# Kiripiro/leaffliction

Hardware: AMD Instinct MI355X
Metric: 224x224 images/sec train (higher is better)
Workload: dtype f32; 1 GPU; leaf_cnn base train step (configs[1]: img 224, batch 256/GPU, fp32, 8 classes, AdamW+clipnorm+EMA, in-model augmentation); per_gpu_batch=256, global_batch=256, img_size=224, parallelism=dp1

## Files before the change

leaffliction_amd/csrc/lf_conv.hip:

```cpp
#include <type_traits>

#include "lf_common.h"

namespace {

typedef float f32x16 __attribute__((ext_vector_type(16)));
typedef float f32x4 __attribute__((ext_vector_type(4)));

constexpr int kThreads = 256;

__device__ __forceinline__ float pro_apply(float v, float sc, float sh, int relu) {
    v = fmaf(v, sc, sh);
    return relu ? fmaxf(v, 0.f) : v;
}

typedef float lf_f4 __attribute__((ext_vector_type(4)));
constexpr unsigned kBufOob = 0xffffffffu;
__device__ __forceinline__ __amdgpu_buffer_rsrc_t buf_rsrc(const float* base, unsigned bytes) {
    return __builtin_amdgcn_make_buffer_rsrc(const_cast<float*>(base), 0, bytes, 0x00020000);
}
__device__ __forceinline__ float4 buf_load4(__amdgpu_buffer_rsrc_t r, unsigned off) {
    const lf_f4 v = __builtin_bit_cast(lf_f4, __builtin_amdgcn_raw_buffer_load_b128(r, off, 0, 0));
    return make_float4(v.x, v.y, v.z, v.w);
}
__device__ __forceinline__ float buf_load1(__amdgpu_buffer_rsrc_t r, unsigned off) {
    return __builtin_bit_cast(float, __builtin_amdgcn_raw_buffer_load_b32(r, off, 0, 0));
}

struct ConvArgs {
    const float* x;
    const float* w;
    const float* wino_u;
    float* y;
    const float* in_scale;
    const float* in_shift;
    int n, cin, cout, h, wd;
    int tiles_x, tiles_y;
    int in_relu;
    int accumulate;
    int vec_ok;
    int stack;
    float* stat_part;
    const float* stat_pivot;
    long long stat_tiles;
    const float* stat_mask_y;
    const float* mask_scale;
    const float* mask_shift;
    int mask_relu;
};

using lf::half_sum32;
using lf::row_sum16;

__device__ __forceinline__ void wino_filter(const float (&g)[9], float (&u)[16]) {
    float t[4][3];
#pragma unroll
    for (int c = 0; c < 3; ++c) {
        const float s = g[c] + g[6 + c];
        t[0][c] = g[c];
        t[1][c] = (s + g[3 + c]) * 0.5f;
        t[2][c] = (s - g[3 + c]) * 0.5f;
        t[3][c] = g[6 + c];
    }
#pragma unroll
    for (int r = 0; r < 4; ++r) {
        const float s = t[r][0] + t[r][2];
        u[r * 4 + 0] = t[r][0];
        u[r * 4 + 1] = (s + t[r][1]) * 0.5f;
        u[r * 4 + 2] = (s - t[r][1]) * 0.5f;
        u[r * 4 + 3] = t[r][2];
    }
}
__device__ __forceinline__ void wino_input(const float (&d)[16], float (&v)[16]) {
    float t[16];
#pragma unroll
    for (int c = 0; c < 4; ++c) {
        t[0 + c] = d[0 + c] - d[8 + c];
        t[4 + c] = d[4 + c] + d[8 + c];
        t[8 + c] = d[8 + c] - d[4 + c];
        t[12 + c] = d[4 + c] - d[12 + c];
    }
#pragma unroll
    for (int r = 0; r < 4; ++r) {
        v[r * 4 + 0] = t[r * 4 + 0] - t[r * 4 + 2];
        v[r * 4 + 1] = t[r * 4 + 1] + t[r * 4 + 2];
        v[r * 4 + 2] = t[r * 4 + 2] - t[r * 4 + 1];
        v[r * 4 + 3] = t[r * 4 + 1] - t[r * 4 + 3];
    }
}
__device__ __forceinline__ void wino_output(const float (&m)[16], float (&y)[4]) {
    float b[2][4];
#pragma unroll
    for (int c = 0; c < 4; ++c) {
        b[0][c] = m[0 + c] + m[4 + c] + m[8 + c];
        b[1][c] = m[4 + c] - m[8 + c] - m[12 + c];
    }
#pragma unroll
    for (int r = 0; r < 2; ++r) {
        y[r * 2 + 0] = b[r][0] + b[r][1] + b[r][2];
        y[r * 2 + 1] = b[r][1] - b[r][2] - b[r][3];
    }
}

constexpr int kMaxProC = 512;

template <int TW, int TH, int HALO, bool STK>
struct ConvTile {
    int bz, by, tile;
    int tx0, ty0, n;
    int imgA, gyA0, ra;
    bool imgA_ok, imgB_ok;

    __device__ __forceinline__ explicit ConvTile(const ConvArgs& p) {
        const unsigned gxy = gridDim.x * gridDim.y, gtotal = gxy * gridDim.z;
        const unsigned bflat = blockIdx.x + gridDim.x * (blockIdx.y + gridDim.y * blockIdx.z);
        const unsigned xk = bflat & 7u, xfloor = gtotal >> 3, xrem = gtotal & 7u;
        const unsigned wid_flat = xk * xfloor + (xk < xrem ? xk : xrem) + (bflat >> 3);
        bz = (int)(wid_flat / gxy);
        by = (int)((wid_flat - (unsigned)bz * gxy) / gridDim.x);
        tile = (int)(wid_flat - (unsigned)bz * gxy - (unsigned)by * gridDim.x);
        tx0 = (tile % p.tiles_x) * TW;
        ty0 = (tile / p.tiles_x) * TH;
        n = bz * p.stack;
        imgA = ty0 / p.h;
        gyA0 = ty0 - imgA * p.h;
        ra = min(TH, p.h - gyA0);
        imgA_ok = imgA < p.stack && n + imgA < p.n;
        imgB_ok = STK && imgA + 1 < p.stack && n + imgA + 1 < p.n;
    }

    __device__ __forceinline__ bool patch_row(int py, int h, int& img, int& gy) const {
        if (py < ra + 2 * HALO) {
            img = imgA;
            gy = gyA0 - HALO + py;
            return imgA_ok && gy >= 0 && gy < h;
        }
        img = imgA + 1;
        gy = py - (ra + 2 * HALO) - HALO;
        return imgB_ok && ra < TH && gy >= 0 && gy < h && gy < TH - ra + HALO;
    }
};

template <int TW, int TH, int HALO, bool STK, int kKC>
struct PatchStage {
    static constexpr int PW = TW + 2 * HALO, PH = TH + 2 * HALO + (STK ? 2 * HALO : 0), PP = PW * PH;
    static constexpr int TW4 = TW / 4;
    static constexpr int NVI = kKC * PH * TW4, IPT = (NVI + kThreads - 1) / kThreads;
    static constexpr int NHI = kKC * PH * 2 * HALO, HPT = (NHI + kThreads - 1) / kThreads;
    static_assert(TW % 4 == 0, "float4 patch rows");

    size_t hw;
    float4 pv[IPT];
    float ph[HPT > 0 ? HPT : 1];
    unsigned pg[IPT], pl[IPT];
    unsigned hg[HPT > 0 ? HPT : 1], hl[HPT > 0 ? HPT : 1];
    unsigned okmask = 0;

    __device__ __forceinline__ PatchStage(const ConvArgs& p, const ConvTile<TW, TH, HALO, STK>& t, float* lsc, int tid) {
        if (p.in_scale != nullptr) {
            for (int c = tid; c < p.cin && c < kMaxProC; c += kThreads) {
                lsc[c] = p.in_scale[c];
                lsc[kMaxProC + c] = p.in_shift[c];
            }
        }
        hw = (size_t)p.h * p.wd;
        const unsigned uhw = (unsigned)hw;
#pragma unroll
        for (int i = 0; i < IPT; ++i) {
            const int e = tid + i * kThreads;
            const int kc = e / (PH * TW4), rem = e - kc * (PH * TW4);
            const int py = rem / TW4, slot = rem - py * TW4;
            int img, gy;
            const bool ok = t.patch_row(py, p.h, img, gy) && e < NVI;
            pg[i] = ok ? 4u * ((unsigned)(img * p.cin + kc) * uhw + (unsigned)gy * (unsigned)p.wd + (unsigned)(t.tx0 + 4 * slot)) : kBufOob;
            pl[i] = (unsigned)(kc * PP + py * PW + HALO + 4 * slot) | ((unsigned)kc << 16);
            okmask |= (ok ? 1u : 0u) << i;
        }
#pragma unroll
        for (int i = 0; i < HPT; ++i) {
            const int e = tid + i * kThreads;
            const int kc = e / (PH * 2), rem = e - kc * (PH * 2);
            const int py = rem >> 1, side = rem & 1;
            const int gx = side ? t.tx0 + TW : t.tx0 - 1;
            int img, gy;
            const bool ok = t.patch_row(py, p.h, img, gy) && e < NHI && gx >= 0 && gx < p.wd;
            hg[i] = ok ? 4u * ((unsigned)(img * p.cin + kc) * uhw + (unsigned)gy * (unsigned)p.wd + (unsigned)gx) : kBufOob;
            hl[i] = (unsigned)(kc * PP + py * PW + (side ? PW - 1 : 0)) | ((unsigned)kc << 16);
            okmask |= (ok ? 1u : 0u) << (16 + i);
        }
    }

    __device__ __forceinline__ void load(const ConvArgs& p, const float* xin, int c0) {
        const __amdgpu_buffer_rsrc_t rx = buf_rsrc(
            xin + (size_t)c0 * hw,
            4u * (unsigned)((STK ? (p.stack - 1) * p.cin : 0) + min(kKC, p.cin - c0)) * (unsigned)hw);
#pragma unroll
        for (int i = 0; i < IPT; ++i) pv[i] = buf_load4(rx, pg[i]);
#pragma unroll
        for (int i = 0; i < HPT; ++i) ph[i] = buf_load1(rx, hg[i]);
    }

    __device__ __forceinline__ void store(const ConvArgs& p, float* lp, const float* lsc, int c0, int tid) const {
        const bool pro = p.in_scale != nullptr;
        auto pro_sc = [&](int c) { return c < kMaxProC ? lsc[c] : p.in_scale[c]; };
        auto pro_sh = [&](int c) { return c < kMaxProC ? lsc[kMaxProC + c] : p.in_shift[c]; };
#pragma unroll
        for (int i = 0; i < IPT; ++i) {
            if (tid + i * kThreads < NVI) {
                const int kc = (int)(pl[i] >> 16);
                float4 v = pv[i];
                if (pro && (okmask >> i & 1u)) {
                    const float sc = pro_sc(c0 + kc), sh = pro_sh(c0 + kc);
                    v.x = pro_apply(v.x, sc, sh, p.in_relu);
                    v.y = pro_apply(v.y, sc, sh, p.in_relu);
                    v.z = pro_apply(v.z, sc, sh, p.in_relu);
                    v.w = pro_apply(v.w, sc, sh, p.in_relu);
                }
                float* dst = lp + (pl[i] & 0xffffu);
                dst[0] = v.x;
                dst[1] = v.y;
                dst[2] = v.z;
                dst[3] = v.w;
            }
        }
#pragma unroll
        for (int i = 0; i < HPT; ++i) {
            if (tid + i * kThreads < NHI) {
                const int kc = (int)(hl[i] >> 16);
                float v = ph[i];
                if (pro && (okmask >> (16 + i) & 1u))
                    v = pro_apply(v, pro_sc(c0 + kc), pro_sh(c0 + kc), p.in_relu);
                lp[hl[i] & 0xffffu] = v;
            }
        }
    }

    static __device__ __forceinline__ void stage_scalar(const ConvArgs& p, float* lp, const float* xin,
                                                        int tx0, int ty0, int c0, int tid) {
        constexpr int SLOTS = PP <= 64 ? 64 : (PP <= 128 ? 128 : 256);
        constexpr int G = kThreads / SLOTS;
        constexpr int ROUNDS = (PP + SLOTS - 1) / SLOTS;
        const int slot = tid % SLOTS, grp = tid / SLOTS;
        const size_t hw = (size_t)p.h * p.wd;
        const unsigned uhw = (unsigned)hw;
        const bool pro = p.in_scale != nullptr;
#pragma unroll
        for (int r = 0; r < ROUNDS; ++r) {
            const int pos = slot + r * SLOTS;
            if (pos < PP) {
                const int py = pos / PW, px = pos - py * PW;
                const int gy = ty0 + py - HALO, gx = tx0 + px - HALO;
                const bool inb = gy >= 0 && gy < p.h && gx >= 0 && gx < p.wd;
                const unsigned goff = inb ? (unsigned)gy * (unsigned)p.wd + (unsigned)gx : 0u;
#pragma unroll 4
                for (int kc = grp; kc < kKC; kc += G) {
                    const int c = c0 + kc;
                    float v = 0.f;
                    if (inb && c < p.cin) {
                        v = xin[(unsigned)c * uhw + goff];
                        if (pro) v = pro_apply(v, p.in_scale[c], p.in_shift[c], p.in_relu);
                    }
                    lp[kc * PP + pos] = v;
                }
            }
        }
    }
};

template <int WPX, int CT>
__device__ __forceinline__ void write_stat_part(const ConvArgs& p, const float* red, int bz, int tile, int co0,
                                                int tid) {
    __syncthreads();
    const long long tg = (long long)bz * (p.tiles_x * p.tiles_y) + tile;
    for (int c = tid; c < CT; c += kThreads) {
        if (co0 + c >= p.cout) continue;
        float a = 0.f, b = 0.f;
#pragma unroll
        for (int wp = 0; wp < WPX; ++wp) {
            a += red[(wp * CT + c) * 2];
            b += red[(wp * CT + c) * 2 + 1];
        }
        float* dst = p.stat_part + ((size_t)(co0 + c) * (size_t)p.stat_tiles + (size_t)tg) * 2;
        dst[0] = a;
        dst[1] = b;
    }
}

template <int TAPS, int TW, int TH, int WCO, int MB, int WPX, int NB, int kKC, bool STK = false>
__global__ __launch_bounds__(kThreads, (MB * NB * 16 <= 32 ? 3 : 2))
void conv_mfma_kernel(ConvArgs p) {
    constexpr int NPB = TW * TH / 32;
    static_assert(TW * TH % 32 == 0, "tile must be whole 32-pixel blocks");
    static_assert(WCO * WPX == 4 && WPX * NB == NPB, "wave decomposition");
    constexpr int CT = 32 * WCO * MB;
    constexpr int HALO = TAPS == 9 ? 1 : 0;
    using Patch = PatchStage<TW, TH, HALO, STK, kKC>;
    constexpr int PW = Patch::PW, PP = Patch::PP;
    constexpr int PATCH = kKC * PP;
    constexpr int WSZ = kKC * TAPS * CT;
    static_assert(PATCH % 4 == 0, "16-byte aligned weight region");
    constexpr int CT4 = CT / 4, NWI = kKC * TAPS * CT4, WPT = (NWI + kThreads - 1) / kThreads;

    __shared__ __attribute__((aligned(16))) float lds[PATCH + WSZ];
    __shared__ float lsc[2 * kMaxProC];
    float* lp = lds;
    float* lw = lds + PATCH;

    const int tid = threadIdx.x, lane = tid & 63, wid = tid >> 6;
    const int wave_co = wid % WCO, wave_px = wid / WCO;
    const ConvTile<TW, TH, HALO, STK> t(p);
    const int co0 = t.by * CT;
    const size_t hw = (size_t)p.h * p.wd;
    const unsigned uhw = (unsigned)hw;
    const float* xin = p.x + (size_t)t.n * p.cin * hw;

    const int khalf = lane >> 5, j = lane & 31;
    int bbase[NB];
#pragma unroll
    for (int nb = 0; nb < NB; ++nb) {
        const int f = (wave_px * NB + nb) * 32 + j;
        const int r = f / TW, prow = (STK && r >= t.ra) ? r + 2 * HALO : r;
        bbase[nb] = khalf * PP + prow * PW + (f % TW);
    }
    const int abase = khalf * TAPS * CT + wave_co * MB * 32 + j;

    f32x16 acc[MB][NB];
#pragma unroll
    for (int m = 0; m < MB; ++m)
#pragma unroll
        for (int nb = 0; nb < NB; ++nb)
#pragma unroll
            for (int r = 0; r < 16; ++r) acc[m][nb][r] = 0.f;

    auto compute_chunk = [&]() {
#pragma unroll 2
        for (int cp = 0; cp < kKC / 2; ++cp) {
            const float* lwc = lw + abase + 2 * cp * TAPS * CT;
            const float* lpc = lp + 2 * cp * PP;
#pragma unroll
            for (int tap = 0; tap < TAPS; ++tap) {
                const int dy = TAPS == 9 ? tap / 3 : 0, dx = TAPS == 9 ? tap % 3 : 0;
                float a[MB], b[NB];
#pragma unroll
                for (int m = 0; m < MB; ++m) a[m] = lwc[tap * CT + m * 32];
#pragma unroll
                for (int nb = 0; nb < NB; ++nb) b[nb] = lpc[bbase[nb] + dy * PW + dx];
#pragma unroll
                for (int m = 0; m < MB; ++m)
#pragma unroll
                    for (int nb = 0; nb < NB; ++nb)
                        acc[m][nb] = __builtin_amdgcn_mfma_f32_32x32x2f32(a[m], b[nb], acc[m][nb], 0, 0, 0);
            }
        }
    };

    const int nchunks = (p.cin + kKC - 1) / kKC;
    const bool vec = p.vec_ok && (t.tx0 + TW <= p.wd);

    if (vec) {
        float4 wv[WPT];
        constexpr bool kPrefetchW = MB * NB * 16 <= 64;
        Patch patch(p, t, lsc, tid);
        unsigned wg[WPT];
#pragma unroll
        for (int i = 0; i < WPT; ++i) {
            const int e = tid + i * kThreads;
            const int row = e / CT4, col = (e - row * CT4) * 4;
            wg[i] = (e < NWI && co0 + col < p.cout) ? 4u * ((unsigned)row * (unsigned)p.cout + (unsigned)(co0 + col)) : kBufOob;
        }
        auto load_weights = [&](int c0) {
            const __amdgpu_buffer_rsrc_t rw =
                buf_rsrc(p.w + (size_t)c0 * TAPS * p.cout,
                         4u * (unsigned)(min(kKC, p.cin - c0) * TAPS) * (unsigned)p.cout);
#pragma unroll
            for (int i = 0; i < WPT; ++i) wv[i] = buf_load4(rw, wg[i]);
        };
        auto store_chunk = [&](int c0) {
            if (!kPrefetchW) load_weights(c0);
            patch.store(p, lp, lsc, c0, tid);
#pragma unroll
            for (int i = 0; i < WPT; ++i) {
                const int e = tid + i * kThreads;
                if (e < NWI) reinterpret_cast<float4*>(lw)[e] = wv[i];
            }
        };
        patch.load(p, xin, 0);
        if (kPrefetchW) load_weights(0);
        for (int ch = 0; ch < nchunks; ++ch) {
            __syncthreads();
            store_chunk(ch * kKC);
            __syncthreads();
            if (ch + 1 < nchunks) {
                patch.load(p, xin, (ch + 1) * kKC);
                if (kPrefetchW) load_weights((ch + 1) * kKC);
            }
            compute_chunk();
        }
    } else {
        constexpr int WROWS = kKC * TAPS, RPP = kThreads / CT;
        const int wcol = tid % CT, wrow0 = tid / CT;
        const bool wcol_ok = co0 + wcol < p.cout;
        for (int ch = 0; ch < nchunks; ++ch) {
            const int c0 = ch * kKC;
            __syncthreads();
            Patch::stage_scalar(p, lp, xin, t.tx0, t.ty0, c0, tid);
            const int wvalid = (p.cin - c0) * TAPS;
#pragma unroll 4
            for (int row = wrow0; row < WROWS; row += RPP) {
                float v = 0.f;
                if (wcol_ok && row < wvalid)
                    v = p.w[((unsigned)c0 * TAPS + row) * (unsigned)p.cout + (unsigned)(co0 + wcol)];
                lw[row * CT + wcol] = v;
            }
            __syncthreads();
            compute_chunk();
        }
    }

    float* yout = p.y + (size_t)t.n * p.cout * hw;
    const bool stats = p.stat_part != nullptr, masked = p.stat_mask_y != nullptr;
    float* red = lds;
    static_assert(WPX * CT * 2 <= PATCH + WSZ, "stat scratch must fit the staging LDS");
    if (stats) __syncthreads();
    const float* my = masked ? p.stat_mask_y + (size_t)t.n * p.cout * hw : nullptr;
    constexpr int RG = TAPS == 1 ? (NB <= 2 ? 4 : 1) : (NB <= 2 ? 16 : 4);
    bool pix_ok[NB];
    unsigned pixc[NB];
#pragma unroll
    for (int nb = 0; nb < NB; ++nb) {
        const int f = (wave_px * NB + nb) * 32 + j;
        const int r = f / TW, ox = t.tx0 + f % TW;
        const bool in_a = r < t.ra;
        const int oy = in_a ? t.gyA0 + r : r - t.ra;
        pix_ok[nb] = (in_a ? t.imgA_ok : t.imgB_ok) && oy < p.h && ox < p.wd;
        pixc[nb] = pix_ok[nb] ? (unsigned)((in_a ? t.imgA : t.imgA + 1) * p.cout) * uhw +
                                    (unsigned)oy * (unsigned)p.wd + (unsigned)ox
                              : 0u;
    }
#pragma unroll
    for (int m = 0; m < MB; ++m) {
#pragma unroll
        for (int rg = 0; rg < 16; rg += RG) {
            float oldv[RG][NB], yv[RG][NB];
            if (p.accumulate) {
#pragma unroll
                for (int rr = 0; rr < RG; ++rr) {
                    const int r = rg + rr;
                    const int co = co0 + (wave_co * MB + m) * 32 + 4 * khalf + (r & 3) + 8 * (r >> 2);
                    const float* src = yout + (size_t)min(co, p.cout - 1) * hw;
#pragma unroll
                    for (int nb = 0; nb < NB; ++nb) oldv[rr][nb] = src[pixc[nb]];
                }
            }
            if (masked) {
#pragma unroll
                for (int rr = 0; rr < RG; ++rr) {
                    const int r = rg + rr;
                    const int co = co0 + (wave_co * MB + m) * 32 + 4 * khalf + (r & 3) + 8 * (r >> 2);
                    const float* src = my + (size_t)min(co, p.cout - 1) * hw;
#pragma unroll
                    for (int nb = 0; nb < NB; ++nb) yv[rr][nb] = src[pixc[nb]];
                }
            }
#pragma unroll
            for (int rr = 0; rr < RG; ++rr) {
                const int r = rg + rr;
                const int cl = (wave_co * MB + m) * 32 + 4 * khalf + (r & 3) + 8 * (r >> 2);
                const int co = co0 + cl;
                const bool co_ok = co < p.cout;
                float* dst = yout + (size_t)co * hw;
#pragma unroll
                for (int nb = 0; nb < NB; ++nb) {
                    if (p.accumulate) acc[m][nb][r] += oldv[rr][nb];
                    if (co_ok && pix_ok[nb])
                        dst[pixc[nb]] = acc[m][nb][r];
                }
                if (!stats) continue;
                float s1 = 0.f, s2 = 0.f;
                if (!masked) {
                    const float pv = (p.stat_pivot != nullptr && co_ok) ? p.stat_pivot[co] : 0.f;
#pragma unroll
                    for (int nb = 0; nb < NB; ++nb)
                        lf::stat_accumulate(acc[m][nb][r], pix_ok[nb], false, pv, 0.f, 0.f, 0.f, 0, s1, s2);
                } else {
                    const float msc = p.mask_scale[min(co, p.cout - 1)], msh = p.mask_shift[min(co, p.cout - 1)];
#pragma unroll
                    for (int nb = 0; nb < NB; ++nb)
                        lf::stat_accumulate(acc[m][nb][r], co_ok && pix_ok[nb], true, 0.f, yv[rr][nb], msc, msh,
                                            p.mask_relu, s1, s2);
                }
                s1 = half_sum32(s1);
                s2 = half_sum32(s2);
                if (j == 31) {
                    red[(wave_px * CT + cl) * 2] = s1;
                    red[(wave_px * CT + cl) * 2 + 1] = s2;
                }
            }
        }
    }
    if (stats) write_stat_part<WPX, CT>(p, red, t.bz, t.tile, co0, tid);
}

template <int TW, int TH, int MB, int NB, bool STK>
__global__ __launch_bounds__(kThreads, 2)
void conv_wino_kernel(ConvArgs p) {
    constexpr int kKC = 8, WPX = 4;
    constexpr int TXN = TW / 2, NT = TXN * (TH / 2);
    static_assert(TH % 2 == 0, "F(2x2,3x3): even tile");
    static_assert(WPX * NB * 16 >= NT, "wave decomposition");
    constexpr int CT = 16 * MB;
    constexpr int kUP = 20;
    using Patch = PatchStage<TW, TH, 1, STK, kKC>;
    constexpr int PW = Patch::PW, PP = Patch::PP;
    constexpr int PATCH = kKC * PP;
    constexpr int WSZ = kKC * CT * kUP;
    static_assert(PATCH % 4 == 0, "16-byte aligned U region");

    __shared__ __attribute__((aligned(16))) float lds[PATCH + WSZ];
    __shared__ float lsc[2 * kMaxProC];
    float* lp = lds;
    float* lw = lds + PATCH;

    const int tid = threadIdx.x, lane = tid & 63, wave_px = tid >> 6;
    const ConvTile<TW, TH, 1, STK> t(p);
    const int co0 = t.by * CT;
    const size_t hw = (size_t)p.h * p.wd;
    const unsigned uhw = (unsigned)hw;
    const float* xin = p.x + (size_t)t.n * p.cin * hw;

    const int wq = lane >> 4, wl = lane & 15;
    int vbase[NB];
    const int ubase = (wq * CT + wl) * kUP;
    f32x4 wacc[MB][NB][16];
#pragma unroll
    for (int nb = 0; nb < NB; ++nb) {
        const int tt = min((wave_px * NB + nb) * 16 + wl, NT - 1);
        const int r0 = 2 * (tt / TXN), prow = (STK && r0 >= t.ra) ? r0 + 2 : r0;
        vbase[nb] = wq * PP + prow * PW + 2 * (tt % TXN);
    }
#pragma unroll
    for (int m = 0; m < MB; ++m)
#pragma unroll
        for (int nb = 0; nb < NB; ++nb)
#pragma unroll
            for (int q = 0; q < 16; ++q) wacc[m][nb][q] = f32x4{0.f, 0.f, 0.f, 0.f};

    auto compute_chunk = [&]() {
#pragma unroll
        for (int s = 0; s < kKC / 4; ++s) {
            float u[MB][16];
#pragma unroll
            for (int m = 0; m < MB; ++m) {
                const float4* us = reinterpret_cast<const float4*>(lw + ubase + (4 * s * CT + m * 16) * kUP);
#pragma unroll
                for (int q4 = 0; q4 < 4; ++q4) {
                    const float4 v4 = us[q4];
                    u[m][4 * q4 + 0] = v4.x;
                    u[m][4 * q4 + 1] = v4.y;
                    u[m][4 * q4 + 2] = v4.z;
                    u[m][4 * q4 + 3] = v4.w;
                }
            }
#pragma unroll
            for (int nb = 0; nb < NB; ++nb) {
                const float* src = lp + vbase[nb] + 4 * s * PP;
                float d[16], v[16];
#pragma unroll
                for (int r = 0; r < 4; ++r) {
                    const float2 lo = *reinterpret_cast<const float2*>(src + r * PW);
                    const float2 hi = *reinterpret_cast<const float2*>(src + r * PW + 2);
                    d[r * 4 + 0] = lo.x;
                    d[r * 4 + 1] = lo.y;
                    d[r * 4 + 2] = hi.x;
                    d[r * 4 + 3] = hi.y;
                }
                wino_input(d, v);
#pragma unroll
                for (int m = 0; m < MB; ++m)
#pragma unroll
                    for (int q = 0; q < 16; ++q)
                        wacc[m][nb][q] = __builtin_amdgcn_mfma_f32_16x16x4f32(u[m][q], v[q], wacc[m][nb][q], 0, 0, 0);
            }
        }
    };

    constexpr int KSTEP = kThreads / (4 * CT), UPT = kKC / KSTEP;
    static_assert(kThreads % (4 * CT) == 0 && kKC % KSTEP == 0, "whole channels per pass");
    const int ukc = tid / (4 * CT), uco = (tid >> 2) % CT, uq4 = tid & 3;
    const unsigned ustep = 64u * KSTEP * (unsigned)p.cout;
    const unsigned ugo = co0 + uco < p.cout ? 4u * (((unsigned)ukc * (unsigned)p.cout + (unsigned)(co0 + uco)) * 16u + 4u * (unsigned)uq4) : 0x80000000u;
    float* const ulds = lw + (ukc * CT + uco) * kUP + 4 * uq4;
    float4 uv[UPT];
    auto load_u = [&](int c0) {
        const __amdgpu_buffer_rsrc_t ru =
            buf_rsrc(p.wino_u + (size_t)c0 * p.cout * 16, 64u * (unsigned)min(kKC, p.cin - c0) * (unsigned)p.cout);
#pragma unroll
        for (int i = 0; i < UPT; ++i) uv[i] = buf_load4(ru, ugo + (unsigned)i * ustep);
    };
    auto store_u = [&]() {
#pragma unroll
        for (int i = 0; i < UPT; ++i) *reinterpret_cast<float4*>(ulds + i * KSTEP * CT * kUP) = uv[i];
    };

    const int nchunks = (p.cin + kKC - 1) / kKC;
    const bool vec = p.vec_ok && (t.tx0 + TW <= p.wd);

    if (vec) {
        Patch patch(p, t, lsc, tid);
        patch.load(p, xin, 0);
        for (int ch = 0; ch < nchunks; ++ch) {
            __syncthreads();
            load_u(ch * kKC);
            patch.store(p, lp, lsc, ch * kKC, tid);
            store_u();
            __syncthreads();
            if (ch + 1 < nchunks) patch.load(p, xin, (ch + 1) * kKC);
            compute_chunk();
        }
    } else {
        for (int ch = 0; ch < nchunks; ++ch) {
            const int c0 = ch * kKC;
            __syncthreads();
            Patch::stage_scalar(p, lp, xin, t.tx0, t.ty0, c0, tid);
            load_u(c0);
            store_u();
            __syncthreads();
            compute_chunk();
        }
    }

    float* yout = p.y + (size_t)t.n * p.cout * hw;
    const bool stats = p.stat_part != nullptr, masked = p.stat_mask_y != nullptr;
    float* red = lds;
    static_assert(WPX * CT * 2 <= PATCH + WSZ, "stat scratch must fit the staging LDS");
    if (stats) __syncthreads();
    const float* my = masked ? p.stat_mask_y + (size_t)t.n * p.cout * hw : nullptr;
    const bool y2 = (p.wd & 1) == 0 && (reinterpret_cast<size_t>(p.y) & 7) == 0;
    bool pok[NB][4];
    unsigned pofs[NB][4];
#pragma unroll
    for (int nb = 0; nb < NB; ++nb) {
        const int tt = (wave_px * NB + nb) * 16 + wl;
        const int r0 = 2 * (tt / TXN), ox = t.tx0 + 2 * (tt % TXN);
        const bool in_a = r0 < t.ra;
        const int oy = in_a ? t.gyA0 + r0 : r0 - t.ra;
        const bool img_ok = tt < NT && (in_a ? t.imgA_ok : t.imgB_ok);
        const unsigned base = (unsigned)((in_a ? t.imgA : t.imgA + 1) * p.cout) * uhw;
#pragma unroll
        for (int q = 0; q < 4; ++q) {
            const int py = oy + (q >> 1), px = ox + (q & 1);
            pok[nb][q] = img_ok && py < p.h && px < p.wd;
            pofs[nb][q] = pok[nb][q] ? base + (unsigned)py * (unsigned)p.wd + (unsigned)px : 0u;
        }
    }
#pragma unroll
    for (int m = 0; m < MB; ++m) {
#pragma unroll
        for (int i = 0; i < 4; ++i) {
            const int cl = m * 16 + 4 * wq + i;
            const int co = co0 + cl;
            const bool co_ok = co < p.cout;
            const size_t cofs = (size_t)min(co, p.cout - 1) * hw;
            float out[NB][4], oldv[NB][4], yv[NB][4];
#pragma unroll
            for (int nb = 0; nb < NB; ++nb) {
                float mm[16];
#pragma unroll
                for (int q = 0; q < 16; ++q) mm[q] = wacc[m][nb][q][i];
                wino_output(mm, out[nb]);
                if (p.accumulate) {
#pragma unroll
                    for (int q = 0; q < 4; ++q) oldv[nb][q] = yout[cofs + pofs[nb][q]];
                }
                if (masked) {
#pragma unroll
                    for (int q = 0; q < 4; ++q) yv[nb][q] = my[cofs + pofs[nb][q]];
                }
            }
#pragma unroll
            for (int nb = 0; nb < NB; ++nb) {
                if (p.accumulate) {
#pragma unroll
                    for (int q = 0; q < 4; ++q) out[nb][q] += oldv[nb][q];
                }
                if (co_ok) {
#pragma unroll
                    for (int r = 0; r < 2; ++r) {
                        float* dst = yout + cofs + pofs[nb][2 * r];
                        if (y2 && pok[nb][2 * r] && pok[nb][2 * r + 1]) {
                            *reinterpret_cast<float2*>(dst) = make_float2(out[nb][2 * r], out[nb][2 * r + 1]);
                        } else {
                            if (pok[nb][2 * r]) dst[0] = out[nb][2 * r];
                            if (pok[nb][2 * r + 1]) yout[cofs + pofs[nb][2 * r + 1]] = out[nb][2 * r + 1];
                        }
                    }
                }
            }
            if (!stats) continue;
            float s1 = 0.f, s2 = 0.f;
            if (!masked) {
                const float pv = (p.stat_pivot != nullptr && co_ok) ? p.stat_pivot[co] : 0.f;
#pragma unroll
                for (int nb = 0; nb < NB; ++nb)
#pragma unroll
                    for (int q = 0; q < 4; ++q)
                        lf::stat_accumulate(out[nb][q], pok[nb][q], false, pv, 0.f, 0.f, 0.f, 0, s1, s2);
            } else {
                const float msc = p.mask_scale[min(co, p.cout - 1)], msh = p.mask_shift[min(co, p.cout - 1)];
#pragma unroll
                for (int nb = 0; nb < NB; ++nb)
#pragma unroll
                    for (int q = 0; q < 4; ++q)
                        lf::stat_accumulate(out[nb][q], co_ok && pok[nb][q], true, 0.f, yv[nb][q], msc, msh, p.mask_relu,
                                            s1, s2);
            }
            s1 = row_sum16(s1);
            s2 = row_sum16(s2);
            if (wl == 0) {
                red[(wave_px * CT + cl) * 2] = s1;
                red[(wave_px * CT + cl) * 2 + 1] = s2;
            }
        }
    }
    if (stats) write_stat_part<WPX, CT>(p, red, t.bz, t.tile, co0, tid);
}

struct WgradArgs {
    const float* x;
    const float* dy;
    float* part;
    const float* in_scale;
    const float* in_shift;
    int n, cin, cout, h, wd;
    int tiles_x, tiles_y, items, items_per_split;
    int in_relu;
    int vec_ok;
    const float* bn_y;
    const float* bn_alpha;
    const float* bn_add;
    const float* bn_coef;
    float* dy_out;
    int bn_relu;
};

__device__ __forceinline__ float bn_dy1(float g, float y, float al, float ad, float c0, float c1,
                                        float c2, float c3, float c4, int relu) {
    float dz = fmaf(g, al, ad);
    if (relu && !(fmaf(y, c0, c1) > 0.f)) dz = 0.f;
    return fmaf(c2, dz, fmaf(c3, y, c4));
}

template <int TW, int TH, int WCI, int WCO, int KSPL>
__global__ __launch_bounds__(kThreads, 4) void wgrad_mfma_kernel(WgradArgs p) {
    static_assert(WCI * WCO * KSPL == 4, "wave decomposition");
    static_assert(TH % KSPL == 0 && TW % 4 == 0, "rows split across waves, float4 rows");
    constexpr int PP = (TW * TH) | 1;
    constexpr int CI_T = 32 * WCI, CO_T = 32 * WCO;
    constexpr int XSZ = CI_T * PP, DSZ = CO_T * PP;
    constexpr int RED = KSPL > 1 ? 1024 : 0;
    constexpr int LDSF = XSZ + DSZ > RED ? XSZ + DSZ : RED;
    constexpr int TW4 = TW / 4;
    constexpr int NXI = CI_T * TH * TW4, XPT = (NXI + kThreads - 1) / kThreads;
    constexpr int NDI = CO_T * TH * TW4, DPT = (NDI + kThreads - 1) / kThreads;
    __shared__ float lds[LDSF];
    float* lx = lds;
    float* ld = lds + XSZ;

    const int tid = threadIdx.x, lane = tid & 63, wid = tid >> 6;
    const int w_ci = wid % WCI, w_co = (wid / WCI) % WCO, w_k = wid / (WCI * WCO);
    const int ci0 = blockIdx.y * CI_T, co0 = blockIdx.z * CO_T;
    const int khalf = lane >> 5, j = lane & 31;
    const size_t hw = (size_t)p.h * p.wd;
    const unsigned uhw = (unsigned)hw;

    f32x16 acc;
#pragma unroll
    for (int r = 0; r < 16; ++r) acc[r] = 0.f;

    const int abase = (w_ci * 32 + j) * PP + khalf;
    const int bbase = (w_co * 32 + j) * PP + khalf;
    const bool pro = p.in_scale != nullptr;

    auto compute_item = [&]() {
        constexpr int ROWS = TH / KSPL;
#pragma unroll
        for (int rr = 0; rr < ROWS; ++rr) {
            const int row = w_k * ROWS + rr;
#pragma unroll 2
            for (int xx = 0; xx < TW; xx += 2) {
                const float b = ld[bbase + row * TW + xx];
                const float a = lx[abase + row * TW + xx];
                acc = __builtin_amdgcn_mfma_f32_32x32x2f32(a, b, acc, 0, 0, 0);
            }
        }
    };

    const int first = blockIdx.x * p.items_per_split;
    const int last = min(first + p.items_per_split, p.items);
    const int tiles = p.tiles_x * p.tiles_y;

    if (p.vec_ok) {
        float4 xv[XPT], dv[DPT];
        unsigned xok = 0;
        __shared__ float lsc[kMaxProC / 2];
        if (pro) {
            for (int c = tid; c < CI_T; c += kThreads) {
                const int gc = ci0 + c;
                lsc[c] = gc < p.cin ? p.in_scale[gc] : 1.f;
                lsc[kMaxProC / 4 + c] = gc < p.cin ? p.in_shift[gc] : 0.f;
            }
        }
        const bool bn = p.bn_y != nullptr;
        float4 yv[DPT];
        float dal[DPT], dad[DPT];
        unsigned dok = 0;
        __shared__ float lbn[5 * CO_T];
        if (bn) {
            for (int e = tid; e < 5 * CO_T; e += kThreads) {
                const int kk = e / CO_T, gc = co0 + (e - kk * CO_T);
                lbn[e] = gc < p.cout ? p.bn_coef[(size_t)kk * p.cout + gc] : 0.f;
            }
        }
        auto load_x = [&](int item) {
            const int n = item / tiles, t = item - n * tiles;
            const int tx0 = (t % p.tiles_x) * TW, ty0 = (t / p.tiles_x) * TH;
            const float* xin = p.x + (size_t)n * p.cin * hw;
            xok = 0;
#pragma unroll
            for (int i = 0; i < XPT; ++i) {
                const int e = tid + i * kThreads;
                float4 v = make_float4(0.f, 0.f, 0.f, 0.f);
                const int c = e / (TH * TW4), rem = e - c * (TH * TW4);
                const int py = rem / TW4, slot = rem - py * TW4;
                const int gc = ci0 + c, gy = ty0 + py;
                if (e < NXI && gc < p.cin && gy < p.h) {
                    v = *reinterpret_cast<const float4*>(xin + (unsigned)gc * uhw +
                                                         (unsigned)gy * (unsigned)p.wd + tx0 + 4 * slot);
                    xok |= 1u << i;
                }
                xv[i] = v;
            }
        };
        auto load_d = [&](int item) {
            const int n = item / tiles, t = item - n * tiles;
            const int tx0 = (t % p.tiles_x) * TW, ty0 = (t / p.tiles_x) * TH;
            const float* din = p.dy + (size_t)n * p.cout * hw;
            dok = 0;
#pragma unroll
            for (int i = 0; i < DPT; ++i) {
                const int e = tid + i * kThreads;
                float4 v = make_float4(0.f, 0.f, 0.f, 0.f);
                const int c = e / (TH * TW4), rem = e - c * (TH * TW4);
                const int py = rem / TW4, slot = rem - py * TW4;
                const int gc = co0 + c, gy = ty0 + py;
                if (e < NDI && gc < p.cout && gy < p.h) {
                    v = *reinterpret_cast<const float4*>(din + (unsigned)gc * uhw +
                                                         (unsigned)gy * (unsigned)p.wd + tx0 + 4 * slot);
                    dok |= 1u << i;
                }
                dv[i] = v;
            }
            if (bn) {
                const float* yin = p.bn_y + (size_t)n * p.cout * hw;
#pragma unroll
                for (int i = 0; i < DPT; ++i) {
                    const int e = tid + i * kThreads;
                    float4 v = make_float4(0.f, 0.f, 0.f, 0.f);
                    const int c = e / (TH * TW4), rem = e - c * (TH * TW4);
                    const int py = rem / TW4, slot = rem - py * TW4;
                    if (dok >> i & 1u)
                        v = *reinterpret_cast<const float4*>(yin + (unsigned)(co0 + c) * uhw +
                                                             (unsigned)(ty0 + py) * (unsigned)p.wd + tx0 + 4 * slot);
                    yv[i] = v;
                }
#pragma unroll
                for (int i = 0; i < DPT; ++i) {
                    const int gc = min(co0 + (tid + i * kThreads) / (TH * TW4), p.cout - 1);
                    dal[i] = p.bn_alpha != nullptr ? p.bn_alpha[(size_t)n * p.cout + gc] : 1.f;
                    dad[i] = p.bn_add != nullptr ? p.bn_add[(size_t)n * p.cout + gc] : 0.f;
                }
            }
        };
        auto store_x = [&]() {
#pragma unroll
            for (int i = 0; i < XPT; ++i) {
                const int e = tid + i * kThreads;
                if (e < NXI) {
                    const int c = e / (TH * TW4), rem = e - c * (TH * TW4);
                    const int py = rem / TW4, slot = rem - py * TW4;
                    float4 v = xv[i];
                    if (pro && (xok >> i & 1u)) {
                        const float sc = lsc[c], sh = lsc[kMaxProC / 4 + c];
                        v.x = pro_apply(v.x, sc, sh, p.in_relu);
                        v.y = pro_apply(v.y, sc, sh, p.in_relu);
                        v.z = pro_apply(v.z, sc, sh, p.in_relu);
                        v.w = pro_apply(v.w, sc, sh, p.in_relu);
                    }
                    float* dst = lx + c * PP + py * TW + 4 * slot;
                    dst[0] = v.x;
                    dst[1] = v.y;
                    dst[2] = v.z;
                    dst[3] = v.w;
                }
            }
        };
        auto store_d = [&](int item) {
            const int sn = item / tiles, st = item - sn * tiles;
            const int stx0 = (st % p.tiles_x) * TW, sty0 = (st / p.tiles_x) * TH;
#pragma unroll
            for (int i = 0; i < DPT; ++i) {
                const int e = tid + i * kThreads;
                if (e < NDI) {
                    const int c = e / (TH * TW4), rem = e - c * (TH * TW4);
                    float4 v = dv[i];
                    if (bn && (dok >> i & 1u)) {
                        const float c0 = lbn[c], c1 = lbn[CO_T + c], c2 = lbn[2 * CO_T + c],
                                    c3 = lbn[3 * CO_T + c], c4 = lbn[4 * CO_T + c];
                        v.x = bn_dy1(v.x, yv[i].x, dal[i], dad[i], c0, c1, c2, c3, c4, p.bn_relu);
                        v.y = bn_dy1(v.y, yv[i].y, dal[i], dad[i], c0, c1, c2, c3, c4, p.bn_relu);
                        v.z = bn_dy1(v.z, yv[i].z, dal[i], dad[i], c0, c1, c2, c3, c4, p.bn_relu);
                        v.w = bn_dy1(v.w, yv[i].w, dal[i], dad[i], c0, c1, c2, c3, c4, p.bn_relu);
                        if (blockIdx.y == 0 && p.dy_out != nullptr) {
                            const int py = rem / TW4, slot = rem - py * TW4;
                            *reinterpret_cast<float4*>(p.dy_out + ((size_t)sn * p.cout + co0 + c) * hw +
                                                       (size_t)(sty0 + py) * p.wd + stx0 + 4 * slot) = v;
                        }
                    }
                    float* dst = ld + c * PP + rem * 4;
                    dst[0] = v.x;
                    dst[1] = v.y;
                    dst[2] = v.z;
                    dst[3] = v.w;
                }
            }
        };
        if (first < last) {
            load_x(first);
            load_d(first);
        }
        for (int item = first; item < last; ++item) {
            __syncthreads();
            store_x();
            store_d(item);
            __syncthreads();
            if (item + 1 < last) {
                load_x(item + 1);
                load_d(item + 1);
            }
            compute_item();
        }
    } else {
        constexpr int POS = TW * TH;
        constexpr int SLOTS = POS <= 64 ? 64 : (POS <= 128 ? 128 : 256);
        constexpr int G = kThreads / SLOTS;
        static_assert(POS <= 256, "wgrad tiles are at most 256 positions");
        const int slot = tid % SLOTS, grp = tid / SLOTS;
        const int spy = slot / TW, spx = slot - spy * TW;
        for (int item = first; item < last; ++item) {
            const int n = item / tiles, t = item - n * tiles;
            const int tx0 = (t % p.tiles_x) * TW, ty0 = (t / p.tiles_x) * TH;
            const float* xin = p.x + (size_t)n * p.cin * hw;
            const float* din = p.dy + (size_t)n * p.cout * hw;
            __syncthreads();
            if (slot < POS) {
                const int gy = ty0 + spy, gx = tx0 + spx;
                const bool ok = gy < p.h && gx < p.wd;
                const unsigned off = ok ? (unsigned)gy * (unsigned)p.wd + (unsigned)gx : 0u;
#pragma unroll 4
                for (int c = grp; c < CI_T; c += G) {
                    const int gc = ci0 + c;
                    float v = 0.f;
                    if (ok && gc < p.cin) {
                        v = xin[(unsigned)gc * uhw + off];
                        if (pro) v = pro_apply(v, p.in_scale[gc], p.in_shift[gc], p.in_relu);
                    }
                    lx[c * PP + slot] = v;
                }
#pragma unroll 4
                for (int c = grp; c < CO_T; c += G) {
                    const int gc = co0 + c;
// ... 1029 lines not shown
```

Before: 6209 images/sec.

## Double-buffer Winograd conv LDS with direct buffer-to-LDS U loads and swizzle

Restructures the Winograd conv main loop to double-buffer both the input patch and the transformed-weight (U) tiles in LDS. U is loaded straight from global memory into LDS with buffer_load ... lds via inline asm, which removes the register round-trip and drops one barrier per chunk. The padded U stride is replaced with an XOR swizzle to avoid bank conflicts. The patch store now reads per-channel affine coefficients from LDS, re-staging them every kMaxProC channels, and epilogue reads of the accumulate and mask inputs are hoisted and vectorised. LDS use roughly doubles, which may reduce occupancy, and the inline asm that manipulates M0 is fragile.

```diff
diff --git a/leaffliction_amd/csrc/lf_conv.hip b/leaffliction_amd/csrc/lf_conv.hip
--- a/leaffliction_amd/csrc/lf_conv.hip
+++ b/leaffliction_amd/csrc/lf_conv.hip
@@ -156,34 +156,44 @@
     unsigned hg[HPT > 0 ? HPT : 1], hl[HPT > 0 ? HPT : 1];
     unsigned okmask = 0;
 
+    static __device__ __forceinline__ void stage_coef(const ConvArgs& p, float* lsc, int c0, int tid) {
+        for (int c = tid; c < kMaxProC; c += kThreads) {
+            const bool in = c0 + c < p.cin;
+            lsc[c] = in ? p.in_scale[c0 + c] : 0.f;
+            lsc[kMaxProC + c] = in ? p.in_shift[c0 + c] : 0.f;
+        }
+    }
+    static __device__ __forceinline__ void restage_coef(const ConvArgs& p, float* lsc, int c0, int tid) {
+        if (p.in_scale != nullptr && c0 != 0 && (c0 & (kMaxProC - 1)) == 0) {
+            __syncthreads();
+            stage_coef(p, lsc, c0, tid);
+            __syncthreads();
+        }
+    }
+
     __device__ __forceinline__ PatchStage(const ConvArgs& p, const ConvTile<TW, TH, HALO, STK>& t, float* lsc, int tid) {
-        if (p.in_scale != nullptr) {
-            for (int c = tid; c < p.cin && c < kMaxProC; c += kThreads) {
-                lsc[c] = p.in_scale[c];
-                lsc[kMaxProC + c] = p.in_shift[c];
-            }
-        }
+        if (p.in_scale != nullptr) stage_coef(p, lsc, 0, tid);
         hw = (size_t)p.h * p.wd;
         const unsigned uhw = (unsigned)hw;
 #pragma unroll
         for (int i = 0; i < IPT; ++i) {
-            const int e = tid + i * kThreads;
+            const int e = (tid + i * kThreads) % NVI;
             const int kc = e / (PH * TW4), rem = e - kc * (PH * TW4);
             const int py = rem / TW4, slot = rem - py * TW4;
             int img, gy;
-            const bool ok = t.patch_row(py, p.h, img, gy) && e < NVI;
+            const bool ok = t.patch_row(py, p.h, img, gy);
             pg[i] = ok ? 4u * ((unsigned)(img * p.cin + kc) * uhw + (unsigned)gy * (unsigned)p.wd + (unsigned)(t.tx0 + 4 * slot)) : kBufOob;
             pl[i] = (unsigned)(kc * PP + py * PW + HALO + 4 * slot) | ((unsigned)kc << 16);
             okmask |= (ok ? 1u : 0u) << i;
         }
 #pragma unroll
         for (int i = 0; i < HPT; ++i) {
-            const int e = tid + i * kThreads;
+            const int e = (tid + i * kThreads) % (NHI > 0 ? NHI : 1);
             const int kc = e / (PH * 2), rem = e - kc * (PH * 2);
             const int py = rem >> 1, side = rem & 1;
             const int gx = side ? t.tx0 + TW : t.tx0 - 1;
             int img, gy;
-            const bool ok = t.patch_row(py, p.h, img, gy) && e < NHI && gx >= 0 && gx < p.wd;
+            const bool ok = t.patch_row(py, p.h, img, gy) && gx >= 0 && gx < p.wd;
             hg[i] = ok ? 4u * ((unsigned)(img * p.cin + kc) * uhw + (unsigned)gy * (unsigned)p.wd + (unsigned)gx) : kBufOob;
             hl[i] = (unsigned)(kc * PP + py * PW + (side ? PW - 1 : 0)) | ((unsigned)kc << 16);
             okmask |= (ok ? 1u : 0u) << (16 + i);
@@ -200,38 +210,54 @@
         for (int i = 0; i < HPT; ++i) ph[i] = buf_load1(rx, hg[i]);
     }
 
-    __device__ __forceinline__ void store(const ConvArgs& p, float* lp, const float* lsc, int c0, int tid) const {
-        const bool pro = p.in_scale != nullptr;
-        auto pro_sc = [&](int c) { return c < kMaxProC ? lsc[c] : p.in_scale[c]; };
-        auto pro_sh = [&](int c) { return c < kMaxProC ? lsc[kMaxProC + c] : p.in_shift[c]; };
-#pragma unroll
-        for (int i = 0; i < IPT; ++i) {
-            if (tid + i * kThreads < NVI) {
-                const int kc = (int)(pl[i] >> 16);
-                float4 v = pv[i];
-                if (pro && (okmask >> i & 1u)) {
-                    const float sc = pro_sc(c0 + kc), sh = pro_sh(c0 + kc);
-                    v.x = pro_apply(v.x, sc, sh, p.in_relu);
-                    v.y = pro_apply(v.y, sc, sh, p.in_relu);
-                    v.z = pro_apply(v.z, sc, sh, p.in_relu);
-                    v.w = pro_apply(v.w, sc, sh, p.in_relu);
-                }
+    static constexpr int kCoefGroup = 2;
+    __device__ __forceinline__ void store(const ConvArgs& p, float* lp, const float* lsc, int c0) const {
+        if (p.in_scale != nullptr) {
+            const float* cf = lsc + (c0 & (kMaxProC - 1));
+#pragma unroll
+            for (int g = 0; g < IPT; g += kCoefGroup) {
+                float sc[kCoefGroup], sh[kCoefGroup];
+#pragma unroll
+                for (int i = g; i < g + kCoefGroup && i < IPT; ++i) {
+                    const bool ok = okmask >> i & 1u;
+                    const float c = cf[pl[i] >> 16], h = cf[kMaxProC + (pl[i] >> 16)];
+                    sc[i - g] = ok ? c : 0.f;
+                    sh[i - g] = ok ? h : 0.f;
+                }
+#pragma unroll
+                for (int i = g; i < g + kCoefGroup && i < IPT; ++i) {
+                    float* dst = lp + (pl[i] & 0xffffu);
+                    dst[0] = pro_apply(pv[i].x, sc[i - g], sh[i - g], p.in_relu);
+                    dst[1] = pro_apply(pv[i].y, sc[i - g], sh[i - g], p.in_relu);
+                    dst[2] = pro_apply(pv[i].z, sc[i - g], sh[i - g], p.in_relu);
+                    dst[3] = pro_apply(pv[i].w, sc[i - g], sh[i - g], p.in_relu);
+                }
+            }
+#pragma unroll
+            for (int g = 0; g < HPT; g += kCoefGroup) {
+                float sc[kCoefGroup], sh[kCoefGroup];
+#pragma unroll
+                for (int i = g; i < g + kCoefGroup && i < HPT; ++i) {
+                    const bool ok = okmask >> (16 + i) & 1u;
+                    const float c = cf[hl[i] >> 16], h = cf[kMaxProC + (hl[i] >> 16)];
+                    sc[i - g] = ok ? c : 0.f;
+                    sh[i - g] = ok ? h : 0.f;
+                }
+#pragma unroll
+                for (int i = g; i < g + kCoefGroup && i < HPT; ++i)
+                    lp[hl[i] & 0xffffu] = pro_apply(ph[i], sc[i - g], sh[i - g], p.in_relu);
+            }
+        } else {
+#pragma unroll
+            for (int i = 0; i < IPT; ++i) {
                 float* dst = lp + (pl[i] & 0xffffu);
-                dst[0] = v.x;
-                dst[1] = v.y;
-                dst[2] = v.z;
-                dst[3] = v.w;
-            }
-        }
-#pragma unroll
-        for (int i = 0; i < HPT; ++i) {
-            if (tid + i * kThreads < NHI) {
-                const int kc = (int)(hl[i] >> 16);
-                float v = ph[i];
-                if (pro && (okmask >> (16 + i) & 1u))
-                    v = pro_apply(v, pro_sc(c0 + kc), pro_sh(c0 + kc), p.in_relu);
-                lp[hl[i] & 0xffffu] = v;
-            }
+                dst[0] = pv[i].x;
+                dst[1] = pv[i].y;
+                dst[2] = pv[i].z;
+                dst[3] = pv[i].w;
+            }
+#pragma unroll
+            for (int i = 0; i < HPT; ++i) lp[hl[i] & 0xffffu] = ph[i];
         }
     }
 
@@ -377,7 +403,8 @@
         };
         auto store_chunk = [&](int c0) {
             if (!kPrefetchW) load_weights(c0);
-            patch.store(p, lp, lsc, c0, tid);
+            Patch::restage_coef(p, lsc, c0, tid);
+            patch.store(p, lp, lsc, c0);
 #pragma unroll
             for (int i = 0; i < WPT; ++i) {
                 const int e = tid + i * kThreads;
@@ -509,17 +536,15 @@
     static_assert(TH % 2 == 0, "F(2x2,3x3): even tile");
     static_assert(WPX * NB * 16 >= NT, "wave decomposition");
     constexpr int CT = 16 * MB;
-    constexpr int kUP = 20;
     using Patch = PatchStage<TW, TH, 1, STK, kKC>;
     constexpr int PW = Patch::PW, PP = Patch::PP;
     constexpr int PATCH = kKC * PP;
-    constexpr int WSZ = kKC * CT * kUP;
-    static_assert(PATCH % 4 == 0, "16-byte aligned U region");
-
-    __shared__ __attribute__((aligned(16))) float lds[PATCH + WSZ];
-    __shared__ float lsc[2 * kMaxProC];
-    float* lp = lds;
-    float* lw = lds + PATCH;
+    constexpr int WSZ = kKC * CT * 16;
+
+    __shared__ __attribute__((aligned(16))) float lds[2 * WSZ + 2 * PATCH + 2 * kMaxProC];
+    float* const lw = lds;
+    float* const lp = lds + 2 * WSZ;
+    float* const lsc = lds + 2 * WSZ + 2 * PATCH;
 
     const int tid = threadIdx.x, lane = tid & 63, wave_px = tid >> 6;
     const ConvTile<TW, TH, 1, STK> t(p);
@@ -530,7 +555,7 @@
 
     const int wq = lane >> 4, wl = lane & 15;
     int vbase[NB];
-    const int ubase = (wq * CT + wl) * kUP;
+    const int ubase = (wq * CT + wl) * 16, usw = (wl >> 2) & 3;
     f32x4 wacc[MB][NB][16];
 #pragma unroll
     for (int nb = 0; nb < NB; ++nb) {
@@ -545,16 +570,18 @@
 #pragma unroll
             for (int q = 0; q < 16; ++q) wacc[m][nb][q] = f32x4{0.f, 0.f, 0.f, 0.f};
 
-    auto compute_chunk = [&]() {
+    auto compute_chunk = [&](int buf) {
+        const float* lwb = lw + buf * WSZ;
+        const float* lpb = lp + buf * PATCH;
 #pragma unroll
         for (int s = 0; s < kKC / 4; ++s) {
             float u[MB][16];
 #pragma unroll
             for (int m = 0; m < MB; ++m) {
-                const float4* us = reinterpret_cast<const float4*>(lw + ubase + (4 * s * CT + m * 16) * kUP);
+                const float4* us = reinterpret_cast<const float4*>(lwb + ubase + (4 * s * CT + m * 16) * 16);
 #pragma unroll
                 for (int q4 = 0; q4 < 4; ++q4) {
-                    const float4 v4 = us[q4];
+                    const float4 v4 = us[q4 ^ usw];
                     u[m][4 * q4 + 0] = v4.x;
                     u[m][4 * q4 + 1] = v4.y;
                     u[m][4 * q4 + 2] = v4.z;
@@ -563,7 +590,7 @@
             }
 #pragma unroll
             for (int nb = 0; nb < NB; ++nb) {
-                const float* src = lp + vbase[nb] + 4 * s * PP;
+                const float* src = lpb + vbase[nb] + 4 * s * PP;
                 float d[16], v[16];
 #pragma unroll
                 for (int r = 0; r < 4; ++r) {
@@ -586,56 +613,83 @@
 
     constexpr int KSTEP = kThreads / (4 * CT), UPT = kKC / KSTEP;
     static_assert(kThreads % (4 * CT) == 0 && kKC % KSTEP == 0, "whole channels per pass");
-    const int ukc = tid / (4 * CT), uco = (tid >> 2) % CT, uq4 = tid & 3;
+    const int ukc = tid / (4 * CT), uco = (tid >> 2) % CT, uq4 = (tid & 3) ^ ((uco >> 2) & 3);
     const unsigned ustep = 64u * KSTEP * (unsigned)p.cout;
     const unsigned ugo = co0 + uco < p.cout ? 4u * (((unsigned)ukc * (unsigned)p.cout + (unsigned)(co0 + uco)) * 16u + 4u * (unsigned)uq4) : 0x80000000u;
-    float* const ulds = lw + (ukc * CT + uco) * kUP + 4 * uq4;
-    float4 uv[UPT];
-    auto load_u = [&](int c0) {
-        const __amdgpu_buffer_rsrc_t ru =
-            buf_rsrc(p.wino_u + (size_t)c0 * p.cout * 16, 64u * (unsigned)min(kKC, p.cin - c0) * (unsigned)p.cout);
-#pragma unroll
-        for (int i = 0; i < UPT; ++i) uv[i] = buf_load4(ru, ugo + (unsigned)i * ustep);
+    typedef unsigned u32x4 __attribute__((ext_vector_type(4)));
+    auto load_u = [&](int c0, int buf) {
+        const size_t ubase_g = reinterpret_cast<size_t>(p.wino_u + (size_t)c0 * p.cout * 16);
+        const u32x4 ru = {(unsigned)ubase_g, (unsigned)(ubase_g >> 32) & 0xffffu,
+                          64u * (unsigned)min(kKC, p.cin - c0) * (unsigned)p.cout, 0x00020000u};
+        const unsigned dst = __builtin_amdgcn_readfirstlane(
+            (unsigned)reinterpret_cast<size_t>((__attribute__((address_space(3))) float*)(lw + buf * WSZ + wave_px * 256)));
+#pragma unroll
+        for (int i = 0; i < UPT; ++i) {
+            unsigned keep;
+            asm volatile(
+                "s_mov_b32 %0, m0\n\t"
+                "s_mov_b32 m0, %3\n\t"
+                "s_nop 0\n\t"
+                "buffer_load_dwordx4 %1, %2, 0 offen lds\n\t"
+                "s_mov_b32 m0, %0"
+                : "=&s"(keep)
+                : "v"(ugo + (unsigned)i * ustep), "s"(ru), "s"(dst + (unsigned)(i * KSTEP * CT * 64))
+                : "memory");
+        }
     };
-    auto store_u = [&]() {
-#pragma unroll
-        for (int i = 0; i < UPT; ++i) *reinterpret_cast<float4*>(ulds + i * KSTEP * CT * kUP) = uv[i];
-    };
+    auto u_arrived = [] { asm volatile("s_waitcnt vmcnt(0)" ::: "memory"); };
 
     const int nchunks = (p.cin + kKC - 1) / kKC;
     const bool vec = p.vec_ok && (t.tx0 + TW <= p.wd);
 
     if (vec) {
         Patch patch(p, t, lsc, tid);
+        load_u(0, 0);
         patch.load(p, xin, 0);
+        __syncthreads();
         for (int ch = 0; ch < nchunks; ++ch) {
+            Patch::restage_coef(p, lsc, ch * kKC, tid);
+            patch.store(p, lp + (ch & 1) * PATCH, lsc, ch * kKC);
+            u_arrived();
             __syncthreads();
-            load_u(ch * kKC);
-            patch.store(p, lp, lsc, ch * kKC, tid);
-            store_u();
-            __syncthreads();
-            if (ch + 1 < nchunks) patch.load(p, xin, (ch + 1) * kKC);
-            compute_chunk();
+            if (ch + 1 < nchunks) {
+                load_u((ch + 1) * kKC, (ch + 1) & 1);
+                patch.load(p, xin, (ch + 1) * kKC);
+            }
+            compute_chunk(ch & 1);
         }
     } else {
         for (int ch = 0; ch < nchunks; ++ch) {
             const int c0 = ch * kKC;
+            load_u(c0, ch & 1);
+            Patch::stage_scalar(p, lp + (ch & 1) * PATCH, xin, t.tx0, t.ty0, c0, tid);
+            u_arrived();
             __syncthreads();
-            Patch::stage_scalar(p, lp, xin, t.tx0, t.ty0, c0, tid);
-            load_u(c0);
-            store_u();
-            __syncthreads();
-            compute_chunk();
+            compute_chunk(ch & 1);
         }
     }
 
     float* yout = p.y + (size_t)t.n * p.cout * hw;
     const bool stats = p.stat_part != nullptr, masked = p.stat_mask_y != nullptr;
     float* red = lds;
-    static_assert(WPX * CT * 2 <= PATCH + WSZ, "stat scratch must fit the staging LDS");
+    static_assert(WPX * CT * 2 <= 2 * WSZ, "stat scratch must fit the staging LDS");
     if (stats) __syncthreads();
     const float* my = masked ? p.stat_mask_y + (size_t)t.n * p.cout * hw : nullptr;
     const bool y2 = (p.wd & 1) == 0 && (reinterpret_cast<size_t>(p.y) & 7) == 0;
+    const bool my2 = y2 && (reinterpret_cast<size_t>(p.stat_mask_y) & 7) == 0;
+    auto read4 = [&](const float* src, bool pairs, const bool (&ok)[4], const unsigned (&ofs)[4], float (&v)[4]) {
+        if (pairs) {
+#pragma unroll
+            for (int r = 0; r < 2; ++r) {
+                const float2 v2 = *reinterpret_cast<const float2*>(src + (ok[2 * r] && ok[2 * r + 1] ? ofs[2 * r] : 0u));
+                v[2 * r] = v2.x;
+                v[2 * r + 1] = v2.y;
+            }
+        } else {
+#pragma unroll
+            for (int q = 0; q < 4; ++q) v[q] = src[ofs[q]];
+        }
+    };
     bool pok[NB][4];
     unsigned pofs[NB][4];
 #pragma unroll
@@ -662,20 +716,20 @@
             const bool co_ok = co < p.cout;
             const size_t cofs = (size_t)min(co, p.cout - 1) * hw;
             float out[NB][4], oldv[NB][4], yv[NB][4];
+            if (p.accumulate) {
+#pragma unroll
+                for (int nb = 0; nb < NB; ++nb) read4(yout + cofs, y2, pok[nb], pofs[nb], oldv[nb]);
+            }
+            if (masked) {
+#pragma unroll
+                for (int nb = 0; nb < NB; ++nb) read4(my + cofs, my2, pok[nb], pofs[nb], yv[nb]);
+            }
 #pragma unroll
             for (int nb = 0; nb < NB; ++nb) {
                 float mm[16];
 #pragma unroll
                 for (int q = 0; q < 16; ++q) mm[q] = wacc[m][nb][q][i];
                 wino_output(mm, out[nb]);
-                if (p.accumulate) {
-#pragma unroll
-                    for (int q = 0; q < 4; ++q) oldv[nb][q] = yout[cofs + pofs[nb][q]];
-                }
-                if (masked) {
-#pragma unroll
-                    for (int q = 0; q < 4; ++q) yv[nb][q] = my[cofs + pofs[nb][q]];
-                }
             }
 #pragma unroll
             for (int nb = 0; nb < NB; ++nb) {
```

Measured after the change: 6227 images/sec, median of 6. No clear change (+0.3%).
